# joaospinto/sip_optimal_control

Hardware: AMD Instinct MI355X
Metric: Riccati sweeps/sec (backward+forward) (higher is better)
Workload: dtype f64

## Files before the change

### __graft_entry__.py

```python
import os
import re
import subprocess
import sys

ROOT = os.path.dirname(os.path.abspath(__file__))
CSRC = os.path.join(ROOT, "sip_optimal_control_amd", "csrc")
LIBDIR = os.path.join(ROOT, "sip_optimal_control_amd", "lib")
HIPCC = os.environ.get("HIPCC", "/opt/rocm/bin/hipcc")


def _digest(paths, extra=()):
    import hashlib
    h = hashlib.sha256()
    for x in extra:
        h.update(("\0arg:" + x).encode())
    for path in sorted(set(paths), key=lambda q: os.path.relpath(q, ROOT)):
        h.update(("\0file:" + os.path.relpath(path, ROOT) + "\0").encode())
        with open(path, "rb") as f:
            h.update(f.read())
    return h.hexdigest()


def _stale(target, digest):
    side = target + ".srchash"
# ... 205 lines not shown
    return _host_build(out, [src, os.path.join(ROOT, "tests", "cpp", "test_dropin.cpp"), hdr,
                             os.path.join(ROOT, "include", "sip_lqr_amd.h")],
                       ["g++", "-std=c++17", "-O2", "-D__HIP_PLATFORM_AMD__", src,
                        "-I", os.path.join(ROOT, "include"), "-I", os.path.join(rocm, "include"),
                        "-L", LIBDIR, "-lsip_lqr_amd", "-L", os.path.join(rocm, "lib"), "-lamdhip64",
                        "-Wl,-rpath,$ORIGIN/../sip_optimal_control_amd/lib",
                        "-Wl,-rpath," + os.path.join(rocm, "lib"), "-o", out], force)


def build_callback_provider_test(force=False):
    src = os.path.join(ROOT, "tests", "cpp", "test_callback_provider.cpp")
    hdrs = [os.path.join(ROOT, "include", "sip_optimal_control_amd", h)
            for h in ("callback_provider_dropin.hpp", "lqr_dropin.hpp")]
    out = os.path.join(ROOT, "tests", "cpp", "test_callback_provider")
    rocm = os.environ.get("ROCM_PATH", "/opt/rocm")
    return _host_build(out, [src] + hdrs + [os.path.join(ROOT, "include", h) for h in ("sip_kkt_amd.h", "sip_lqr_amd.h")],
                       ["g++", "-std=c++17", "-O2", "-D__HIP_PLATFORM_AMD__", src,
                        "-I", os.path.join(ROOT, "include"), "-I", os.path.join(rocm, "include"),
                        "-L", LIBDIR, "-lsip_lqr_amd", "-L", os.path.join(rocm, "lib"), "-lamdhip64",
                        "-Wl,-rpath,$ORIGIN/../../sip_optimal_control_amd/lib",
                        "-Wl,-rpath," + os.path.join(rocm, "lib"), "-o", out], force)


def build_kkt_lds_test(force=False):
    src = os.path.join(ROOT, "tests", "cpp", "test_kkt_lds.cpp")
    hdrs = [os.path.join(CSRC, h) for h in ("kkt_kernels.hpp", "kkt_chain_kernels.hpp", "kkt_theta_kernels.hpp",
                                            "kkt_theta_chain_kernels.hpp", "kkt_chain_launch.hpp")]
    out = os.path.join(ROOT, "build", "test_kkt_lds")
    os.makedirs(os.path.dirname(out), exist_ok=True)
    return _host_build(out, [src] + hdrs,
                       [HIPCC, "-x", "hip", "--cuda-host-only", "-std=c++17", "-O1", src, "-o", out], force)


def build_kkt_plan_test(force=False):
    src = os.path.join(ROOT, "tests", "cpp", "test_kkt_plan.cpp")
    hdrs = [os.path.join(CSRC, h) for h in ("kkt_plan.hpp", "kkt_first_order_kernels.hpp", "kkt_kernels.hpp",
                                            "kkt_chain_kernels.hpp", "kkt_theta_kernels.hpp",
                                            "kkt_theta_chain_kernels.hpp", "kkt_chain_launch.hpp")]
    hdrs += [os.path.join(ROOT, "include", h) for h in ("sip_kkt_amd.h", "sip_lqr_amd.h")]
    out = os.path.join(ROOT, "build", "test_kkt_plan")
    os.makedirs(os.path.dirname(out), exist_ok=True)
    return _host_build(out, [src] + hdrs,
                       [HIPCC, "-x", "hip", "--offload-arch=gfx950", "-std=c++17", "-O1", src, "-o", out], force)


def build_tree_plan_test(force=False):
    src = os.path.join(ROOT, "tests", "cpp", "test_tree_plan.cpp")
    hdrs = [os.path.join(CSRC, h) for h in ("tree_plan.hpp", "generic_plan.hpp", "table_packer.hpp", "stream_fill.hpp",
                                            "tree_generic.hpp", "tree_lds.hpp", "tree_qw16_launch.hpp",
                                            "tree_schedule.hpp")]
    hdrs.append(os.path.join(ROOT, "include", "sip_lqr_amd.h"))
    out = os.path.join(ROOT, "build", "test_tree_plan")
    os.makedirs(os.path.dirname(out), exist_ok=True)
    return _host_build(out, [src] + hdrs,
                       [HIPCC, "-x", "hip", "--cuda-host-only", "-std=c++17", "-O1", src,
                        "-L", LIBDIR, "-lsip_lqr_amd", "-Wl,-rpath,$ORIGIN/../sip_optimal_control_amd/lib",
                        "-o", out], force)


def build_residual_cols_shape_test(force=False):
    src = os.path.join(ROOT, "tests", "cpp", "test_residual_cols_shape.cpp")
    out = os.path.join(ROOT, "build", "test_residual_cols_shape")
    os.makedirs(os.path.dirname(out), exist_ok=True)
    return _host_build(out, [src, os.path.join(CSRC, "residual_cols_shape.hpp")],
                       ["g++", "-std=c++17", "-O1", "-Wall", "-I", CSRC, src, "-o", out], force)


def build_tree_residual_cols_shape_test(force=False):
    src = os.path.join(ROOT, "tests", "cpp", "test_tree_residual_cols_shape.cpp")
    out = os.path.join(ROOT, "build", "test_tree_residual_cols_shape")
    os.makedirs(os.path.dirname(out), exist_ok=True)
    return _host_build(out, [src, os.path.join(CSRC, "tree_residual_cols_shape.hpp")],
                       ["g++", "-std=c++17", "-O1", "-Wall", "-I", CSRC, src, "-o", out], force)


def build_oracle():
    sys.path.insert(0, ROOT)
    from oracle import oracle
    return oracle.build()


def build():
    build_hip()
    build_rccl()
    build_group_test()
    build_dropin_test()
    build_dropin_split_test()
    build_callback_provider_test()
    build_kkt_lds_test()
    build_kkt_plan_test()
    build_tree_plan_test()
    build_residual_cols_shape_test()
    build_tree_residual_cols_shape_test()
    build_oracle()
    sys.path.insert(0, ROOT)
    import sip_optimal_control_amd
    from sip_optimal_control_amd._lib import load_library
    load_library()


def smoke():
    sys.path.insert(0, ROOT)
    import numpy as np
    import torch
    from sip_optimal_control_amd import BatchedChainLQR, ChainShape, synthetic
    from oracle import oracle
    assert torch.cuda.is_available(), "smoke() needs a GPU"
    from sip_optimal_control_amd._lib import load_library
    print("library:", load_library().sip_lqr_version().decode())
    shape = ChainShape(n=12, m=4, T=10)
    batch = 37
    mats, vecs = synthetic.make_chain_batch(shape, batch, seed=3, device="cuda:0", cross_term=0.01)
    solver = BatchedChainLQR(shape.n, shape.m, shape.T, batch, device="cuda:0")
    sol, gains, status = solver.factor_solve(mats, vecs)
    torch.cuda.synchronize()
    ref_sol, ref_gains, ref_status = oracle.chain_batch(shape.n, shape.m, shape.T,
                                                       mats.cpu().numpy(), vecs.cpu().numpy())
    assert (status.cpu().numpy() == ref_status).all(), "status mismatch"
    err = np.abs(sol.cpu().numpy() - ref_sol).max() / np.abs(ref_sol).max()
    gerr = np.abs(gains.cpu().numpy() - ref_gains).max() / np.abs(ref_gains).max()
    assert err < 1e-9 and gerr < 1e-9, (err, gerr)
    print(f"smoke ok: kernel={solver.kernel_name} rel err sol={err:.2e} gains={gerr:.2e}")
# ... 24 lines not shown
```

### sip_optimal_control_amd/csrc/chain_mt16.hip

```cpp
#include "chain_mt16.hpp"
#include "mt16_launch.hpp"

namespace sipamd {

static_assert(mt16::Layout<float, 8>::WSN == kMt16SpillPerNode && mt16::Layout<double, 4>::WSN == kMt16SpillPerNode,
              "the dispatch table sizes the workspace by kMt16SpillPerNode");

#define SIP_MT16_INSTANTIATE(S, M)                                                                           \
  template hipError_t launch_mt16<S, M>(long, int, const void *, const void *, void *, void *, int32_t *,    \
                                        void *, hipStream_t, int, void *);
SIP_MT16_INSTANTIATE(float, 8)
SIP_MT16_INSTANTIATE(float, 4)
SIP_MT16_INSTANTIATE(double, 8)
SIP_MT16_INSTANTIATE(double, 4)

}
```

### sip_optimal_control_amd/csrc/chain_mt16.hpp

```cpp
#pragma once
#include <hip/hip_runtime.h>

#include "mt16_launch.hpp"

#ifdef SIP_MT16_STAMPS
#define SIP_MT16_STAMP_ARG , unsigned long long *__restrict__ stamps
#define SIP_MT16_STAMP(k)                                                                                     \
  do {                                                                                                       \
    const unsigned long long now_ = __builtin_amdgcn_s_memtime();                                            \
    seg_[k] += now_ - last_;                                                                                 \
    last_ = now_;                                                                                            \
  } while (0)
#else
#define SIP_MT16_STAMP_ARG
#define SIP_MT16_STAMP(k)
#endif

namespace sipamd {
namespace mt16 {

constexpr int N = 32;

template <typename S> struct Tr;
template <> struct Tr<float> {
// ... 219 lines not shown
        ig = sel(L.mg[0], i0, sel(L.mg[1], i1, sel(L.mg[2], i2, i3)));
      } else {
        const S t1 = fma_(m10, L.eg[0], L.eg[1]);
        const S t2 = fma_(m20, L.eg[0], fma_(m21, L.eg[1], L.eg[2]));
        const S t3 = fma_(m30, L.eg[0], fma_(m31, L.eg[1], fma_(m32, L.eg[2], L.eg[3])));
        amix = fma_(L.ej[0], L.eg[0], fma_(L.ej[1], t1, fma_(L.ej[2], t2, L.ej[3] * t3)));
        ig = fma_(i0, L.eg[0], fma_(i1, L.eg[1], fma_(i2, L.eg[2], i3 * L.eg[3])));
      }
      const bool diag = L.j == TR::row(L.g, v);
      const S one_d = diag ? S(1) : S(0);
      S bop[TILES], aop[TILES];
#pragma unroll
      for (int Jt = 0; Jt < TILES; ++Jt) {
        const S src = T[I][Jt][v] - (Jt == I ? one_d : S(0));
        const v4 mixed = TR::mfma(amix, src, zero4<S>());
        aop[Jt] = -mixed[0];
        bop[Jt] = mixed[0] * ig;
      }
#pragma unroll
      for (int It = 0; It < TILES; ++It)
#pragma unroll
        for (int Jt = 0; Jt < TILES; ++Jt)
          T[It][Jt] = TR::mfma(aop[It], bop[Jt], T[It][Jt]);
      T[I][I][v] -= S(2) * one_d;
    }
  }
  return fail;
}

template <typename S, int M> struct Layout {
  static constexpr int NODE = N * N + N;
  static constexpr int EDGE = N * N + 2 * N * M + M * M;
  static constexpr int VNODE = 2 * N, VEDGE = M, GAIN = M * N + M;
  static constexpr int WTILES = 3, WSN = WTILES * 256 + N;
  static constexpr int VM = (M + 3) / 4;
  static constexpr bool VEC_LOADS = Tr<S>::ROWS_CONTIGUOUS && (EDGE % 4 == 0);
};

template <typename S, bool VEC>
__device__ __forceinline__ Mat32<S> load32(const rsrc_t r, const unsigned ocol, const unsigned so) {
  constexpr unsigned ES = sizeof(S);
  Mat32<S> m;
#pragma unroll
  for (int I = 0; I < 2; ++I)
#pragma unroll
    for (int J = 0; J < 2; ++J) {
      if constexpr (VEC) {
        m.t[I][J] = Mem<S>::ld4(r, (ocol + (unsigned)(16 * J * N + 16 * I)) * ES, so * ES);
      } else {
#pragma unroll
        for (int v = 0; v < 4; ++v)
          m.t[I][J][v] = Mem<S>::ld(r, (ocol + (unsigned)(16 * J * N + 16 * I + Tr<S>::RSTEP * v)) * ES, so * ES);
      }
    }
  return m;
}

#ifndef SIP_MT16_WAVES_F32
#define SIP_MT16_WAVES_F32 4
#endif
template <typename S, int M> struct Waves {
  static constexpr int value = sizeof(S) == 8 ? 2 : M > 8 ? 3 : SIP_MT16_WAVES_F32;
};

template <typename S, int M>
__global__ __launch_bounds__(64) __attribute__((amdgpu_waves_per_eu(Waves<S, M>::value, Waves<S, M>::value)))
void chain_factor_solve_mt16(
    const S *__restrict__ mats, const S *__restrict__ vecs, S *__restrict__ sol, S *__restrict__ gains,
    S *__restrict__ wsp, int *__restrict__ status, const long batch, const int T SIP_MT16_STAMP_ARG) {
  constexpr bool FACTOR = false;
// ... 45 lines not shown
```

### sip_optimal_control_amd/csrc/chain_mt16_solve.hip

```cpp
#include "chain_mt16_solve.hpp"
#include "mt16_launch.hpp"

namespace sipamd {

static_assert(mt16::Layout<float, 8>::WSN == kMt16SpillPerNode, "the spill the factor sweep left");
static_assert(mt16_col_workspace_scalars(3, 8, 5) == 4 * 5 * (mt16::N + 8), "cws[node][column][g | k]");

#define SIP_MT16_SOLVE_INSTANTIATE(S, M)                                                                     \
  template hipError_t launch_mt16_solve<S, M>(long, int, const void *, const void *, void *, void *, void *, \
                                              const void *, void *, const int32_t *, int, long, hipStream_t); \
  template hipError_t launch_mt16_factor<S, M>(long, int, const void *, void *, int32_t *, void *, void *, hipStream_t);
SIP_MT16_SOLVE_INSTANTIATE(float, 8)
SIP_MT16_SOLVE_INSTANTIATE(float, 4)
SIP_MT16_SOLVE_INSTANTIATE(double, 8)
SIP_MT16_SOLVE_INSTANTIATE(double, 4)

}
```

### sip_optimal_control_amd/csrc/chain_mt16_solve.hpp

```cpp
#pragma once
#include "chain_mt16.hpp"

namespace sipamd {
namespace mt16 {

template <typename S> __device__ __forceinline__ void mul_t_pair(const Mat32<S> &U, const Pair<S> &X, Pair<S> &acc) {
#pragma unroll
  for (int R = 0; R < 2; ++R)
#pragma unroll
    for (int v = 0; v < 4; ++v)
#pragma unroll
      for (int I = 0; I < 2; ++I)
        acc.t[I] = Tr<S>::mfma(U.t[R][I][v], X.t[R][v], acc.t[I]);
}

template <typename S, int M>
__global__ __launch_bounds__(64) __attribute__((amdgpu_waves_per_eu(2)))
void chain_solve_mt16(const S *__restrict__ mats, const S *__restrict__ vecs_cols, S *sol_cols, S *gains, S *wsp,
                      const S *__restrict__ gfac, S *cws, const int *__restrict__ status, const long batch,
                      const int T, const int ncols, const long col_stride) {
  static_assert(M >= 1 && M <= 16, "controls live in registers 0 .. VM - 1 of the four lane groups: 16 tile rows");
  using TR = Tr<S>;
  using v4 = typename TR::v4;
  using LY = Layout<S, M>;
  constexpr int STG = LY::NODE + LY::EDGE, VSTG = LY::VNODE + LY::VEDGE, VM = LY::VM;
  constexpr bool VEC = LY::VEC_LOADS;
  constexpr unsigned ES = sizeof(S);
  constexpr int GF = M * M + M;
  constexpr int CW = N + M;
  const long p = blockIdx.x;
  if (p >= batch || status[p] != 0)
    return;
  const int lane = threadIdx.x & 63, j = lane & 15, g = lane >> 4;
  const int acol = ctrl_of_col<S>(j);
  const bool colok = j < ncols;
  const long cj = colok ? j : 0;
  const long mats_len = (long)(T + 1) * LY::NODE + (long)T * LY::EDGE, vecs_len = (long)(T + 1) * LY::VNODE + (long)T * LY::VEDGE;
  const rsrc_t rM = make_rsrc(mats + p * mats_len, mats_len * ES);
  const rsrc_t rG = make_rsrc(gains + p * ((long)T * LY::GAIN), (long)T * LY::GAIN * ES);
  const rsrc_t rW = make_rsrc(wsp + p * ((long)(T + 1) * LY::WSN), (long)(T + 1) * LY::WSN * ES);
  const rsrc_t rF = make_rsrc(gfac + p * ((long)T * GF), (long)T * GF * ES);
  const S *pv = vecs_cols + cj * col_stride + p * vecs_len;
  S *ps = sol_cols + cj * col_stride + p * vecs_len;
  S *pg, *pk;
  long gstride, kstride;
  if (cws != nullptr) {
    pg = cws + (p * (long)(T + 1) * ncols + cj) * CW, gstride = (long)ncols * CW;
    pk = pg + N, kstride = gstride;
  } else {
    pg = wsp + p * ((long)(T + 1) * LY::WSN) + LY::WTILES * 256, gstride = LY::WSN;
    pk = gains + p * ((long)T * LY::GAIN) + M * N, kstride = LY::GAIN;
  }
  const unsigned acolc = (unsigned)(acol < M ? acol : 0);
  const unsigned uj = (unsigned)j, ug = (unsigned)g, r0 = (unsigned)TR::row(g, 0);
  const unsigned ocol = uj * N + r0;
  const unsigned obcol = acolc * N + r0;
  const unsigned orow = r0 * N + uj;
  const unsigned octl = ug * N + uj;
  auto ldM = [&](const unsigned vo, const unsigned so) { return Mem<S>::ld(rM, vo * ES, so * ES); };
  int arow[VM];
  bool aok[VM];
#pragma unroll
  for (int v = 0; v < VM; ++v) {
    const int a = ctrl_of(g, v);
    aok[v] = a < M, arow[v] = a < M ? a : M - 1;
  }

  auto ld_pair = [&](const S *base, const long off) {
    Pair<S> r;
#pragma unroll
    for (int I = 0; I < 2; ++I)
#pragma unroll
      for (int v = 0; v < 4; ++v) {
        const S x = base[off + 16 * I + TR::row(g, v)];
        r.t[I][v] = colok ? x : S(0);
      }
    return r;
  };
  auto st_pair = [&](S *base, const long off, const Pair<S> &x) {
    if (colok) {
#pragma unroll
      for (int I = 0; I < 2; ++I)
#pragma unroll
        for (int v = 0; v < 4; ++v)
          base[off + 16 * I + TR::row(g, v)] = x.t[I][v];
    }
  };
  auto ld_ctl = [&](const S *base, const long off) {
    v4 r = zero4<S>();
#pragma unroll
    for (int v = 0; v < VM; ++v) {
      const S x = base[off + arow[v]];
      r[v] = (colok && aok[v]) ? x : S(0);
    }
    return r;
  };
  auto st_ctl = [&](S *base, const long off, const v4 x) {
#pragma unroll
    for (int v = 0; v < VM; ++v)
      if (colok && aok[v])
        base[off + arow[v]] = x[v];
  };
  auto ld_delta = [&](const int i) {
    Pair<S> r;
#pragma unroll
    for (int I = 0; I < 2; ++I)
#pragma unroll
      for (int v = 0; v < 4; ++v)
        r.t[I][v] = ldM((unsigned)(N * N + 16 * I) + r0 + (unsigned)(TR::RSTEP * v), (unsigned)i * STG);
    return r;
  };
  auto fetch_W = [&](const int i) {
    Mat32<S> W;
    const unsigned sW = (unsigned)i * LY::WSN * ES, vl = (unsigned)lane * 4u * ES;
    W.t[0][0] = Mem<S>::ld4(rW, vl, sW), W.t[1][0] = Mem<S>::ld4(rW, vl + 256u * ES, sW);
    W.t[1][1] = Mem<S>::ld4(rW, vl + 512u * ES, sW);
    const unsigned gq = TR::ROWS_CONTIGUOUS ? (uj >> 2) : (uj & 3u), vq = TR::ROWS_CONTIGUOUS ? (uj & 3u) : (uj >> 2);
    const unsigned ot = (16u * gq + r0) * 4u + vq;
#pragma unroll
    for (int v = 0; v < 4; ++v)
      W.t[0][1][v] = Mem<S>::ld(rW, (ot + (unsigned)((64 + TR::RSTEP * v) * 4)) * ES, sW);
    return W;
  };
  auto t_of = [&](const Pair<S> &c, const Pair<S> &dl, const Pair<S> &v) {
    Pair<S> t;
#pragma unroll
    for (int I = 0; I < 2; ++I)
#pragma unroll
      for (int r = 0; r < 4; ++r)
        t.t[I][r] = fma_(-dl.t[I][r], v.t[I][r], c.t[I][r]);
    return t;
  };

  Mat32<S> W, A;
  Pair<S> B, K, q, c, dl;
  v4 Gm, rv;
  auto fetch_B = [&](const int i) {
    const unsigned sB = (unsigned)i * STG + LY::NODE + N * N;
#pragma unroll
    for (int I = 0; I < 2; ++I) {
      if constexpr (VEC) {
        B.t[I] = Mem<S>::ld4(rM, (obcol + (unsigned)(16 * I)) * ES, sB * ES);
      } else {
#pragma unroll
        for (int v = 0; v < 4; ++v)
          B.t[I][v] = ldM(obcol + (unsigned)(16 * I + TR::RSTEP * v), sB);
      }
      if (acol >= M)
        B.t[I] = zero4<S>();
    }
    rv = ld_ctl(pv, (long)i * VSTG + LY::VNODE);
  };
  auto fetch_G = [&](const int i) {
    Gm = zero4<S>();
#pragma unroll
    for (int v = 0; v < VM; ++v) {
// ... 169 lines not shown
```

### sip_optimal_control_amd/csrc/chain_mt16_sweep_body.hpp

```cpp
#ifndef SIP_MT16_SWEEP_BODY
#error "chain_mt16_sweep_body.hpp is the text of the two kernels of chain_mt16.hpp: include it only where they do"
#endif
  static_assert(M >= 1 && M <= 16, "controls live in registers 0 .. VM - 1 of the four lane groups: 16 tile rows");
#ifdef SIP_MT16_STAMPS
  unsigned long long seg_[16] = {0}, last_ = __builtin_amdgcn_s_memtime();
  const unsigned long long start_ = last_;
#endif
  using TR = Tr<S>;
  using v4 = typename TR::v4;
  using LY = Layout<S, M>;
  constexpr int STG = LY::NODE + LY::EDGE, VSTG = LY::VNODE + LY::VEDGE, VM = LY::VM;
  constexpr bool VEC = LY::VEC_LOADS;
  const long p = blockIdx.x;
  if (p >= batch)
    return;
  LaneT<S> L;
  L.lane = threadIdx.x & 63, L.j = L.lane & 15, L.g = L.lane >> 4;
#pragma unroll
  for (int k = 0; k < 4; ++k) {
    if constexpr (sizeof(S) == 4) {
      L.mg[k] = opaque_mask(L.g == k);
      L.mj[k] = opaque_mask(L.j == TR::row(k, 0));
    } else {
      L.eg[k] = L.g == k ? S(1) : S(0);
      L.ej[k] = L.j == TR::row(k, 0) ? S(1) : S(0);
    }
  }
  const int j = L.j, g = L.g;
  const int acol = ctrl_of_col<S>(j);
  constexpr unsigned ES = sizeof(S);
  const long mats_len = (long)(T + 1) * LY::NODE + (long)T * LY::EDGE, vecs_len = (long)(T + 1) * LY::VNODE + (long)T * LY::VEDGE;
  const rsrc_t rM = make_rsrc(mats + p * mats_len, mats_len * ES), rV = make_rsrc(vecs + p * vecs_len, vecs_len * ES);
  const rsrc_t rS = make_rsrc(sol + p * vecs_len, vecs_len * ES);
  const rsrc_t rG = make_rsrc(gains + p * ((long)T * LY::GAIN), (long)T * LY::GAIN * ES);
  const rsrc_t rW = make_rsrc(wsp + p * ((long)(T + 1) * LY::WSN), (long)(T + 1) * LY::WSN * ES);
  const unsigned acolc = (unsigned)(acol < M ? acol : 0);
  const unsigned uj = (unsigned)j, ug = (unsigned)g, r0 = (unsigned)TR::row(g, 0);
  const unsigned ocol = uj * N + r0;
  const unsigned obcol = acolc * N + r0;
  const unsigned orow = r0 * N + uj;
  const unsigned octl = ug * N + uj;
  constexpr unsigned RS = (unsigned)TR::RSTEP;
  auto ldM = [&](const unsigned vo, const unsigned so) { return Mem<S>::ld(rM, vo * ES, so * ES); };
  auto ldV = [&](const unsigned vo, const unsigned so) { return Mem<S>::ld(rV, vo * ES, so * ES); };

  constexpr int MH = M <= 8 ? 8 : 16;
  __shared__ S s_v[N], s_t[N], s_g[N], s_sd[N], s_sdi[N], s_x[N], s_z[N], s_gs[16], s_h[MH], s_u[MH];
  constexpr int LDM = TR::ROWS_CONTIGUOUS ? 36 : 33;
  __shared__ __attribute__((aligned(16))) S s_m[N * LDM];
  __shared__ __attribute__((aligned(16))) S s_p[16];


  if constexpr (!FACTOR) {
    if (L.lane < MH)
      s_h[L.lane] = S(0), s_u[L.lane] = S(0);
  }
  int stat = 0;
  Mat32<S> W, V;

  auto finish_node = [&](const int i, const S dl0, const S dl1, const S c0, const S c1) {
    if (stat == 0 && __any(!(dl0 > S(0)) || !(dl1 > S(0))))
      stat = 1;
    const S sd0 = TR::sqrt(dl0), sd1 = TR::sqrt(dl1);
    const S sdi0 = S(1) / sd0, sdi1 = S(1) / sd1;
    if (g == 0) {
      s_sd[j] = sd0, s_sd[16 + j] = sd1;
      s_sdi[j] = sdi0, s_sdi[16 + j] = sdi1;
      if constexpr (!FACTOR) {
        s_t[j] = c0 - dl0 * s_v[j];
        s_t[16 + j] = c1 - dl1 * s_v[16 + j];
      }
    }
    SIP_MT16_STAMP(7);
#pragma unroll
// ... 52 lines not shown
      for (int I = 0; I < 2; ++I)
#pragma unroll
        for (int J = 0; J < 2; ++J)
#pragma unroll
          for (int v = 0; v < 4; ++v)
            V.t[I][J][v] *= fr[I][v] * (J == 0 ? fs0 : fs1);
      const bool ffail_scaled = sweep<S, 2, 4>(V.t, L, s_p);
#pragma unroll
      for (int I = 0; I < 2; ++I)
#pragma unroll
        for (int J = 0; J < 2; ++J)
#pragma unroll
          for (int v = 0; v < 4; ++v)
            V.t[I][J][v] *= fr[I][v] * (J == 0 ? fs0 : fs1);
      if (stat == 0 && ffail_scaled)
        stat = 2;
    }
    const bool ffail = SCALE_F ? false : sweep<S, 2, 4>(V.t, L, s_p);
    SIP_MT16_STAMP(9);
    if (stat == 0 && ffail)
      stat = 2;
    {
      const v4 ir[2] = {by_row<S>(s_sdi, 0, g), by_row<S>(s_sdi, 1, g)};
#pragma unroll
      for (int I = 0; I < 2; ++I)
#pragma unroll
        for (int J = 0; J < 2; ++J)
#pragma unroll
          for (int v = 0; v < 4; ++v) {
            const bool dg = I == J && j == TR::row(g, v);
            W.t[I][J][v] = (V.t[I][J][v] + (dg ? S(1) : S(0))) * (ir[I][v] * (J == 0 ? sdi0 : sdi1));
          }
    }
    {
      const unsigned so = (unsigned)i * LY::WSN * ES, vo = (unsigned)L.lane * 4u * ES;
      Mem<S>::st4(W.t[0][0], rW, vo, so);
      Mem<S>::st4(W.t[1][0], rW, vo + 256u * ES, so);
      Mem<S>::st4(W.t[1][1], rW, vo + 512u * ES, so);
    }
    lds_order();
    SIP_MT16_STAMP(10);
  };

  {
    const unsigned sM = (unsigned)T * STG, sV = (unsigned)T * VSTG;
    V = load32<S, VEC>(rM, ocol, sM);
    if constexpr (!FACTOR) {
      const S qT0 = ldV(uj, sV), qT1 = ldV(uj + 16u, sV);
      if (g == 0)
        s_v[j] = qT0, s_v[16 + j] = qT1;
    }
    const S dl0 = ldM(uj + (unsigned)(N * N), sM), dl1 = ldM(uj + (unsigned)(N * N + 16), sM);
    S c0 = S(0), c1 = S(0);
    if constexpr (!FACTOR)
      c0 = ldV(uj + (unsigned)N, sV), c1 = ldV(uj + (unsigned)(N + 16), sV);
    lds_order();
    finish_node(T, dl0, dl1, c0, c1);
  }

  for (int i = T - 1; i >= 0; --i) {
    const unsigned sN = (unsigned)i * STG, sE = sN + LY::NODE, sB = sE + N * N, sMm = sB + N * M, sR = sMm + N * M;
    const unsigned sV = (unsigned)i * VSTG;
    const Mat32<S> A = load32<S, VEC>(rM, ocol, sE);
    const S dl0 = ldM(uj + (unsigned)(N * N), sN), dl1 = ldM(uj + (unsigned)(N * N + 16), sN);
    S c0 = S(0), c1 = S(0), q0 = S(0), q1 = S(0), rv = S(0);
    if constexpr (!FACTOR) {
      c0 = ldV(uj + (unsigned)N, sV), c1 = ldV(uj + (unsigned)(N + 16), sV);
      q0 = ldV(uj, sV), q1 = ldV(uj + 16u, sV), rv = ldV(acolc + (unsigned)LY::VNODE, sV);
    }
    Pair<S> B;
#pragma unroll
    for (int I = 0; I < 2; ++I) {
// ... 1 lines not shown
        B.t[I] = Mem<S>::ld4(rM, (obcol + (unsigned)(16 * I)) * ES, sB * ES);
      } else {
#pragma unroll
        for (int v = 0; v < 4; ++v)
          B.t[I][v] = ldM(obcol + (unsigned)(16 * I) + RS * v, sB);
      }
      if (acol >= M)
        B.t[I] = zero4<S>();
    }
    Pair<S> H;
    v4 G;
#pragma unroll
    for (int v = 0; v < 4; ++v) {
      const int a = ctrl_of(g, v);
      const bool ok = v < VM && a < M;
      if (v < VM) {
        const S h0 = ldM(octl + (unsigned)(4 * v * N), sMm), h1 = ldM(octl + (unsigned)(4 * v * N + 16), sMm);
        const S rr = ldM(acolc * M + ug + (unsigned)(4 * v), sR);
        H.t[0][v] = ok ? h0 : S(0);
        H.t[1][v] = ok ? h1 : S(0);
        G[v] = (ok && acol < M) ? rr : (j == TR::row(g, v) ? S(1) : S(0));
      } else {
        H.t[0][v] = S(0), H.t[1][v] = S(0);
        G[v] = j == TR::row(g, v) ? S(1) : S(0);
      }
    }
    if constexpr (!FACTOR) {
      const v4 tr[2] = {by_row<S>(s_t, 0, g), by_row<S>(s_t, 1, g)};
      S w0 = S(0), w1 = S(0);
      mat_t_vec<S>(W, tr, w0, w1);
      const S g0 = s_v[j] + sum_groups(w0), g1 = s_v[16 + j] + sum_groups(w1);
      if (g == 0) {
        s_g[j] = g0, s_g[16 + j] = g1;
        const unsigned so = ((unsigned)(i + 1) * LY::WSN + LY::WTILES * 256) * ES;
        Mem<S>::st(g0, rW, uj * ES, so);
        Mem<S>::st(g1, rW, (uj + 16u) * ES, so);
      }
    }
    SIP_MT16_STAMP(0);
    Mat32<S> F;
    Pair<S> Z;
#pragma unroll
    for (int I = 0; I < 2; ++I) {
      Z.t[I] = zero4<S>();
#pragma unroll
      for (int J = 0; J < 2; ++J)
        F.t[I][J] = zero4<S>();
    }
#pragma unroll
    for (int R = 0; R < 2; ++R)
#pragma unroll
      for (int v = 0; v < 4; ++v)
#pragma unroll
        for (int I = 0; I < 2; ++I) {
          Z.t[I] = TR::mfma(W.t[R][I][v], B.t[R][v], Z.t[I]);
#pragma unroll
          for (int J = 0; J < 2; ++J)
            F.t[I][J] = TR::mfma(W.t[R][I][v], A.t[R][J][v], F.t[I][J]);
        }
#pragma unroll
    for (int R = 0; R < 2; ++R)
#pragma unroll
      for (int v = 0; v < 4; ++v) {
        G = TR::mfma(B.t[R][v], Z.t[R][v], G);
        H.t[0] = TR::mfma(B.t[R][v], F.t[R][0][v], H.t[0]);
        H.t[1] = TR::mfma(B.t[R][v], F.t[R][1][v], H.t[1]);
      }
// ... 109 lines not shown
    lds_order();
    SIP_MT16_STAMP(5);
    finish_node(i, dl0, dl1, c0, c1);
  }
#ifdef SIP_MT16_STAMPS
  const unsigned long long back_end_ = __builtin_amdgcn_s_memtime();
#endif

  if constexpr (!FACTOR) {
    const v4 tr[2] = {by_row<S>(s_t, 0, g), by_row<S>(s_t, 1, g)};
    S w0 = S(0), w1 = S(0);
    mat_t_vec<S>(W, tr, w0, w1);
    const S g0 = s_v[j] + sum_groups(w0), g1 = s_v[16 + j] + sum_groups(w1);
    if (g == 0) {
      const S x0 = ldV(uj + (unsigned)N, 0u) - ldM(uj + (unsigned)(N * N), 0u) * g0;
      const S x1 = ldV(uj + (unsigned)(N + 16), 0u) - ldM(uj + (unsigned)(N * N + 16), 0u) * g1;
      Mem<S>::st(x0, rS, uj * ES, 0u), Mem<S>::st(x1, rS, (uj + 16u) * ES, 0u);
      Mem<S>::st(g0, rS, (uj + (unsigned)N) * ES, 0u), Mem<S>::st(g1, rS, (uj + (unsigned)(N + 16)) * ES, 0u);
      s_x[j] = x0, s_x[16 + j] = x1;
    }
  }
  if (L.lane == 0)
    status[p] = stat;
  lds_order();

  if constexpr (!FACTOR) {
  Pair<S> KT;
  Mat32<S> AT;
  Pair<S> BT;
  Mat32<S> Wc;
  S kb, gc0, gc1, cc0, cc1, dc0, dc1;
  auto fetch_K = [&](const int i) {
    const unsigned so = (unsigned)i * LY::GAIN * ES;
#pragma unroll
    for (int I = 0; I < 2; ++I)
#pragma unroll
      for (int v = 0; v < 4; ++v)
        KT.t[I][v] = Mem<S>::ld(rG, (r0 * M + acolc + (unsigned)((16 * I + TR::RSTEP * v) * M)) * ES, so);
    kb = Mem<S>::ld(rG, (acolc + (unsigned)(M * N)) * ES, so);
  };
  auto fetch_AB = [&](const int i) {
    const unsigned sE = (unsigned)i * STG + LY::NODE;
#pragma unroll
    for (int I = 0; I < 2; ++I)
#pragma unroll
      for (int v = 0; v < 4; ++v) {
        AT.t[I][0][v] = ldM(orow + (unsigned)((16 * I + TR::RSTEP * v) * N), sE);
        AT.t[I][1][v] = ldM(orow + (unsigned)((16 * I + TR::RSTEP * v) * N + 16), sE);
      }
#pragma unroll
    for (int v = 0; v < VM; ++v) {
      const int a = ctrl_of(g, v);
      const S b0 = ldM(octl + (unsigned)(N * N + 4 * v * N), sE), b1 = ldM(octl + (unsigned)(N * N + 4 * v * N + 16), sE);
      BT.t[0][v] = a < M ? b0 : S(0);
      BT.t[1][v] = a < M ? b1 : S(0);
    }
  };
  auto fetch_W = [&](const int i) {
    const unsigned sN1 = (unsigned)(i + 1) * STG, sV1 = (unsigned)(i + 1) * VSTG, sW = (unsigned)(i + 1) * LY::WSN;
    const unsigned vl = (unsigned)L.lane * 4u * ES;
    Wc.t[0][0] = Mem<S>::ld4(rW, vl, sW * ES), Wc.t[1][0] = Mem<S>::ld4(rW, vl + 256u * ES, sW * ES);
    Wc.t[1][1] = Mem<S>::ld4(rW, vl + 512u * ES, sW * ES);
    {
      const unsigned gq = TR::ROWS_CONTIGUOUS ? (uj >> 2) : (uj & 3u), vq = TR::ROWS_CONTIGUOUS ? (uj & 3u) : (uj >> 2);
      const unsigned ot = (16u * gq + r0) * 4u + vq;
#pragma unroll
      for (int v = 0; v < 4; ++v)
        Wc.t[0][1][v] = Mem<S>::ld(rW, (ot + (unsigned)((64 + TR::RSTEP * v) * 4)) * ES, sW * ES);
    }
    gc0 = Mem<S>::ld(rW, (uj + (unsigned)(LY::WTILES * 256)) * ES, sW * ES);
    gc1 = Mem<S>::ld(rW, (uj + (unsigned)(LY::WTILES * 256 + 16)) * ES, sW * ES);
    cc0 = ldV(uj + (unsigned)N, sV1), cc1 = ldV(uj + (unsigned)(N + 16), sV1);
    dc0 = ldM(uj + (unsigned)(N * N), sN1), dc1 = ldM(uj + (unsigned)(N * N + 16), sN1);
  };
  if (T > 0) {
    fetch_K(0);
    fetch_AB(0);
    fetch_W(0);
  }
  for (int i = 0; i < T; ++i) {
    const bool more = i + 1 < T;
    const v4 xr[2] = {by_row<S>(s_x, 0, g), by_row<S>(s_x, 1, g)};
    S pu = S(0);
#pragma unroll
    for (int I = 0; I < 2; ++I)
#pragma unroll
      for (int v = 0; v < 4; ++v)
        pu = fma_(KT.t[I][v], xr[I][v], pu);
    const S ub = kb + sum_groups(pu);
    if (more)
      fetch_K(i + 1);
    if (g == 0 && acol < M)
      s_u[acol] = ub;
    lds_order();
    S z0 = S(0), z1 = S(0);
    mat_t_vec<S>(AT, xr, z0, z1);
#pragma unroll
    for (int v = 0; v < VM; ++v) {
      const S ur = s_u[ctrl_of(g, v)];
      z0 = fma_(BT.t[0][v], ur, z0);
      z1 = fma_(BT.t[1][v], ur, z1);
    }
    if (more)
      fetch_AB(i + 1);
    z0 = sum_groups(z0), z1 = sum_groups(z1);
    if (g == 0)
// ... 29 lines not shown
```

### sip_optimal_control_amd/csrc/chain_mt16_wide.hip

```cpp
#include "chain_mt16.hpp"
#include "mt16_launch.hpp"

namespace sipamd {

static_assert(mt16::Layout<float, 16>::WSN == kMt16SpillPerNode && mt16::Layout<double, 12>::WSN == kMt16SpillPerNode,
              "the dispatch table sizes the workspace by kMt16SpillPerNode");
static_assert(mt16::Layout<double, 12>::VM == 3 && mt16::Layout<float, 16>::VM == 4, "control registers per lane");

#define SIP_MT16_WIDE_INSTANTIATE(S, M)                                                                      \
  template hipError_t launch_mt16<S, M>(long, int, const void *, const void *, void *, void *, int32_t *,    \
                                        void *, hipStream_t, int, void *);
SIP_MT16_WIDE_INSTANTIATE(float, 16)
SIP_MT16_WIDE_INSTANTIATE(float, 12)
SIP_MT16_WIDE_INSTANTIATE(double, 16)
SIP_MT16_WIDE_INSTANTIATE(double, 12)

}
```

### sip_optimal_control_amd/csrc/chain_mt16_wide_solve.hip

```cpp
#include "chain_mt16_solve.hpp"
#include "mt16_launch.hpp"

namespace sipamd {

static_assert(mt16::Layout<float, 16>::WSN == kMt16SpillPerNode, "the spill the factor sweep left");
static_assert(mt16_col_workspace_scalars(3, 16, 5) == 4 * 5 * (mt16::N + 16), "cws[node][column][g | k]");

#define SIP_MT16_WIDE_SOLVE_INSTANTIATE(S, M)                                                                \
  template hipError_t launch_mt16_solve<S, M>(long, int, const void *, const void *, void *, void *, void *, \
                                              const void *, void *, const int32_t *, int, long, hipStream_t); \
  template hipError_t launch_mt16_factor<S, M>(long, int, const void *, void *, int32_t *, void *, void *, hipStream_t);
SIP_MT16_WIDE_SOLVE_INSTANTIATE(float, 16)
SIP_MT16_WIDE_SOLVE_INSTANTIATE(float, 12)
SIP_MT16_WIDE_SOLVE_INSTANTIATE(double, 16)
SIP_MT16_WIDE_SOLVE_INSTANTIATE(double, 12)

}
```

### sip_optimal_control_amd/csrc/mt16_launch.hpp

```cpp
#pragma once
#include <hip/hip_runtime.h>

#include <cstdint>

namespace sipamd {

template <typename S, int M>
hipError_t launch_mt16(long batch, int T, const void *mats, const void *vecs, void *sol, void *gains,
                       int32_t *status, void *ws, hipStream_t stream, int mode, void *gfac);

constexpr int kMt16SpillPerNode = 3 * 256 + 32;

constexpr int kMt16SolveColumns = 16;
constexpr long mt16_col_workspace_scalars(int T, int m, int ncols) { return (long)(T + 1) * ncols * (32 + m); }
constexpr char kSeparateSuffix[] = " + chain_factor_mt16 + chain_solve_mt16";

template <typename S, int M>
hipError_t launch_mt16_factor(long batch, int T, const void *mats, void *gains, int32_t *status, void *ws, void *gfac,
                              hipStream_t stream);
template <typename S, int M>
hipError_t launch_mt16_solve(long batch, int T, const void *mats, const void *vecs_cols, void *sol_cols, void *gains,
                             void *ws, const void *gfac, void *cws, const int32_t *status, int ncols, long col_stride,
                             hipStream_t stream);

}

#define MT16_ENTRY(DT, S, TAG, M)                                                                            \
  sipamd::with_separate_sweeps({DT, 32, M, "chain_factor_solve_mt16<32," #M ",mfma16x16x4>/" TAG,            \
                                sipamd::kMt16SpillPerNode, &sipamd::launch_mt16<S, M>},                      \
                               {&sipamd::launch_mt16_factor<S, M>, &sipamd::launch_mt16_solve<S, M>,         \
                                sipamd::kSeparateSuffix, sipamd::kMt16SolveColumns, 32 + M})
```

Measured before the change: 13.24 million.

## Pack symmetric diagonal spill tiles for fp32 and hoist per-lane load offsets

Changes the per-node workspace spill of the symmetric W matrix. In fp32 the two diagonal 16x16 tiles are stored packed, keeping only one triangle (160 instead of 256 scalars each), and readers mirror the dropped entries from the transposed position. fp64 keeps the whole-tile layout. Load offsets in the forward sweep are pinned into registers with an empty asm barrier so the constant parts fold into immediates. The aim is less spill traffic and fewer address computations, at the cost of more complex indexing and an out-of-range store offset for dropped elements.

Result: slower. 12.99 million (-1.9%).

```diff
diff --git a/__graft_entry__.py b/__graft_entry__.py
--- a/__graft_entry__.py
+++ b/__graft_entry__.py
@@ -261,6 +261,15 @@
                        [HIPCC, "-x", "hip", "--cuda-host-only", "-std=c++17", "-O1", src, "-o", out], force)
 
 
+def build_mt16_spill_layout_test(force=False):
+    src = os.path.join(ROOT, "tests", "cpp", "test_mt16_spill_layout.cpp")
+    hdrs = [os.path.join(CSRC, h) for h in ("chain_mt16.hpp", "mt16_launch.hpp")]
+    out = os.path.join(ROOT, "build", "test_mt16_spill_layout")
+    os.makedirs(os.path.dirname(out), exist_ok=True)
+    return _host_build(out, [src] + hdrs,
+                       [HIPCC, "-x", "hip", "--cuda-host-only", "-std=c++17", "-O1", src, "-o", out], force)
+
+
 def build_kkt_plan_test(force=False):
     src = os.path.join(ROOT, "tests", "cpp", "test_kkt_plan.cpp")
     hdrs = [os.path.join(CSRC, h) for h in ("kkt_plan.hpp", "kkt_first_order_kernels.hpp", "kkt_kernels.hpp",
@@ -317,6 +326,7 @@
     build_dropin_split_test()
     build_callback_provider_test()
     build_kkt_lds_test()
+    build_mt16_spill_layout_test()
     build_kkt_plan_test()
     build_tree_plan_test()
     build_residual_cols_shape_test()
diff --git a/sip_optimal_control_amd/csrc/chain_mt16.hip b/sip_optimal_control_amd/csrc/chain_mt16.hip
--- a/sip_optimal_control_amd/csrc/chain_mt16.hip
+++ b/sip_optimal_control_amd/csrc/chain_mt16.hip
@@ -3,8 +3,10 @@
 
 namespace sipamd {
 
-static_assert(mt16::Layout<float, 8>::WSN == kMt16SpillPerNode && mt16::Layout<double, 4>::WSN == kMt16SpillPerNode,
-              "the dispatch table sizes the workspace by kMt16SpillPerNode");
+static_assert(mt16::Layout<float, 8>::WSN == mt16::spill_per_node<float>() && mt16::Layout<double, 4>::WSN == mt16::spill_per_node<double>(),
+              "the dispatch table sizes the workspace by mt16::spill_per_node");
+static_assert(mt16::Layout<float, 8>::WSN == 2 * 160 + 256 + 32 && mt16::Layout<double, 4>::WSN == 3 * 256 + 32,
+              "fp32: two packed diagonal tiles and tile (1, 0) | g; fp64: three whole tiles | g");
 
 #define SIP_MT16_INSTANTIATE(S, M)                                                                           \
   template hipError_t launch_mt16<S, M>(long, int, const void *, const void *, void *, void *, int32_t *,    \
diff --git a/sip_optimal_control_amd/csrc/chain_mt16.hpp b/sip_optimal_control_amd/csrc/chain_mt16.hpp
--- a/sip_optimal_control_amd/csrc/chain_mt16.hpp
+++ b/sip_optimal_control_amd/csrc/chain_mt16.hpp
@@ -275,10 +275,64 @@
   static constexpr int NODE = N * N + N;
   static constexpr int EDGE = N * N + 2 * N * M + M * M;
   static constexpr int VNODE = 2 * N, VEDGE = M, GAIN = M * N + M;
-  static constexpr int WTILES = 3, WSN = WTILES * 256 + N;
+  using SP = Spill<Tr<S>::ROWS_CONTIGUOUS>;
+  static constexpr bool PACKED = SP::PACKED;
+  static constexpr int WTILES = SP::WTILES, WSN = SP::WSN;
+  static constexpr int T00 = SP::T00, T10 = SP::T10, T11 = SP::T11, GOFF = SP::GOFF;
+  static __host__ __device__ constexpr bool kept(const int r, const int c) { return SP::kept(r, c); }
+  static __host__ __device__ constexpr int woff(const int r, const int c) { return SP::woff(r, c); }
+  static __host__ __device__ constexpr int roff(const int r, const int c) { return SP::roff(r, c); }
   static constexpr int VM = (M + 3) / 4;
   static constexpr bool VEC_LOADS = Tr<S>::ROWS_CONTIGUOUS && (EDGE % 4 == 0);
 };
+
+constexpr unsigned SPILL_DROPPED = 0x7ffff000u;
+template <typename S, int M> __device__ __forceinline__ unsigned spill_diag_offset(const int j, const int g) {
+  using LY = Layout<S, M>;
+  const int r = Tr<S>::row(g, 0);
+  return LY::kept(r, j) ? (unsigned)LY::woff(r, j) * (unsigned)sizeof(S) : SPILL_DROPPED;
+}
+template <typename S, int M>
+__device__ __forceinline__ void store_spill_W(const Mat32<S> &W, const rsrc_t rW, const unsigned so, const unsigned vdiag,
+                                              const int lane) {
+  using LY = Layout<S, M>;
+  constexpr unsigned ES = sizeof(S);
+  Mem<S>::st4(W.t[0][0], rW, vdiag + (unsigned)LY::T00 * ES, so);
+  Mem<S>::st4(W.t[1][0], rW, (unsigned)lane * 4u * ES + (unsigned)LY::T10 * ES, so);
+  Mem<S>::st4(W.t[1][1], rW, vdiag + (unsigned)LY::T11 * ES, so);
+}
+__device__ __forceinline__ unsigned in_place(unsigned x) {
+  asm volatile("" : "+v"(x));
+  return x;
+}
+template <typename S, int M>
+__device__ __forceinline__ Mat32<S> load_spill_W(const rsrc_t rW, const unsigned so, const int lane, const int j, const int g) {
+  using LY = Layout<S, M>;
+  using TR = Tr<S>;
+  constexpr unsigned ES = sizeof(S);
+  Mat32<S> W;
+  const unsigned vl = in_place((unsigned)lane * 4u * ES);
+  const unsigned vt = in_place((unsigned)LY::roff(TR::row(g, 0), 16 + j) * ES);
+  W.t[1][0] = Mem<S>::ld4(rW, vl + (unsigned)LY::T10 * ES, so);
+#pragma unroll
+  for (int v = 0; v < 4; ++v)
+    W.t[0][1][v] = Mem<S>::ld(rW, vt + (unsigned)(4 * TR::RSTEP * v) * ES, so);
+  if constexpr (LY::PACKED) {
+    const bool kp = LY::kept(TR::row(g, 0), j);
+    const unsigned vd = in_place((unsigned)(kp ? LY::woff(TR::row(g, 0), j) : LY::woff(j, TR::row(g, 0))) * ES);
+    const unsigned step = in_place(kp ? ES : 4u * ES);
+#pragma unroll
+    for (int v = 0; v < 4; ++v) {
+      const unsigned vo = vd + (unsigned)v * step;
+      W.t[0][0][v] = Mem<S>::ld(rW, vo + (unsigned)LY::T00 * ES, so);
+      W.t[1][1][v] = Mem<S>::ld(rW, vo + (unsigned)LY::T11 * ES, so);
+    }
+  } else {
+    W.t[0][0] = Mem<S>::ld4(rW, vl + (unsigned)LY::T00 * ES, so);
+    W.t[1][1] = Mem<S>::ld4(rW, vl + (unsigned)LY::T11 * ES, so);
+  }
+  return W;
+}
 
 template <typename S, bool VEC>
 __device__ __forceinline__ Mat32<S> load32(const rsrc_t r, const unsigned ocol, const unsigned so) {
diff --git a/sip_optimal_control_amd/csrc/chain_mt16_solve.hip b/sip_optimal_control_amd/csrc/chain_mt16_solve.hip
--- a/sip_optimal_control_amd/csrc/chain_mt16_solve.hip
+++ b/sip_optimal_control_amd/csrc/chain_mt16_solve.hip
@@ -3,7 +3,7 @@
 
 namespace sipamd {
 
-static_assert(mt16::Layout<float, 8>::WSN == kMt16SpillPerNode, "the spill the factor sweep left");
+static_assert(mt16::Layout<float, 8>::WSN == mt16::spill_per_node<float>(), "the spill the factor sweep left");
 static_assert(mt16_col_workspace_scalars(3, 8, 5) == 4 * 5 * (mt16::N + 8), "cws[node][column][g | k]");
 
 #define SIP_MT16_SOLVE_INSTANTIATE(S, M)                                                                     \
diff --git a/sip_optimal_control_amd/csrc/chain_mt16_solve.hpp b/sip_optimal_control_amd/csrc/chain_mt16_solve.hpp
--- a/sip_optimal_control_amd/csrc/chain_mt16_solve.hpp
+++ b/sip_optimal_control_amd/csrc/chain_mt16_solve.hpp
@@ -48,7 +48,7 @@
     pg = cws + (p * (long)(T + 1) * ncols + cj) * CW, gstride = (long)ncols * CW;
     pk = pg + N, kstride = gstride;
   } else {
-    pg = wsp + p * ((long)(T + 1) * LY::WSN) + LY::WTILES * 256, gstride = LY::WSN;
+    pg = wsp + p * ((long)(T + 1) * LY::WSN) + LY::GOFF, gstride = LY::WSN;
     pk = gains + p * ((long)T * LY::GAIN) + M * N, kstride = LY::GAIN;
   }
   const unsigned acolc = (unsigned)(acol < M ? acol : 0);
@@ -110,18 +110,7 @@
         r.t[I][v] = ldM((unsigned)(N * N + 16 * I) + r0 + (unsigned)(TR::RSTEP * v), (unsigned)i * STG);
     return r;
   };
-  auto fetch_W = [&](const int i) {
-    Mat32<S> W;
-    const unsigned sW = (unsigned)i * LY::WSN * ES, vl = (unsigned)lane * 4u * ES;
-    W.t[0][0] = Mem<S>::ld4(rW, vl, sW), W.t[1][0] = Mem<S>::ld4(rW, vl + 256u * ES, sW);
-    W.t[1][1] = Mem<S>::ld4(rW, vl + 512u * ES, sW);
-    const unsigned gq = TR::ROWS_CONTIGUOUS ? (uj >> 2) : (uj & 3u), vq = TR::ROWS_CONTIGUOUS ? (uj & 3u) : (uj >> 2);
-    const unsigned ot = (16u * gq + r0) * 4u + vq;
-#pragma unroll
-    for (int v = 0; v < 4; ++v)
-      W.t[0][1][v] = Mem<S>::ld(rW, (ot + (unsigned)((64 + TR::RSTEP * v) * 4)) * ES, sW);
-    return W;
-  };
+  auto fetch_W = [&](const int i) { return load_spill_W<S, M>(rW, (unsigned)i * LY::WSN * ES, lane, j, g); };
   auto t_of = [&](const Pair<S> &c, const Pair<S> &dl, const Pair<S> &v) {
     Pair<S> t;
 #pragma unroll
diff --git a/sip_optimal_control_amd/csrc/chain_mt16_sweep_body.hpp b/sip_optimal_control_amd/csrc/chain_mt16_sweep_body.hpp
--- a/sip_optimal_control_amd/csrc/chain_mt16_sweep_body.hpp
+++ b/sip_optimal_control_amd/csrc/chain_mt16_sweep_body.hpp
@@ -40,6 +40,7 @@
   const unsigned obcol = acolc * N + r0;
   const unsigned orow = r0 * N + uj;
   const unsigned octl = ug * N + uj;
+  const unsigned wdiag = spill_diag_offset<S, M>(j, g);
   constexpr unsigned RS = (unsigned)TR::RSTEP;
   auto ldM = [&](const unsigned vo, const unsigned so) { return Mem<S>::ld(rM, vo * ES, so * ES); };
   auto ldV = [&](const unsigned vo, const unsigned so) { return Mem<S>::ld(rV, vo * ES, so * ES); };
@@ -158,12 +159,7 @@
             W.t[I][J][v] = (V.t[I][J][v] + (dg ? S(1) : S(0))) * (ir[I][v] * (J == 0 ? sdi0 : sdi1));
           }
     }
-    {
-      const unsigned so = (unsigned)i * LY::WSN * ES, vo = (unsigned)L.lane * 4u * ES;
-      Mem<S>::st4(W.t[0][0], rW, vo, so);
-      Mem<S>::st4(W.t[1][0], rW, vo + 256u * ES, so);
-      Mem<S>::st4(W.t[1][1], rW, vo + 512u * ES, so);
-    }
+    store_spill_W<S, M>(W, rW, (unsigned)i * LY::WSN * ES, wdiag, L.lane);
     lds_order();
     SIP_MT16_STAMP(10);
   };
@@ -231,7 +227,7 @@
       const S g0 = s_v[j] + sum_groups(w0), g1 = s_v[16 + j] + sum_groups(w1);
       if (g == 0) {
         s_g[j] = g0, s_g[16 + j] = g1;
-        const unsigned so = ((unsigned)(i + 1) * LY::WSN + LY::WTILES * 256) * ES;
+        const unsigned so = ((unsigned)(i + 1) * LY::WSN + LY::GOFF) * ES;
         Mem<S>::st(g0, rW, uj * ES, so);
         Mem<S>::st(g1, rW, (uj + 16u) * ES, so);
       }
@@ -407,46 +403,41 @@
   S kb, gc0, gc1, cc0, cc1, dc0, dc1;
   auto fetch_K = [&](const int i) {
     const unsigned so = (unsigned)i * LY::GAIN * ES;
+    const unsigned vk = in_place((r0 * M + acolc) * ES), va = in_place(acolc * ES);
 #pragma unroll
     for (int I = 0; I < 2; ++I)
 #pragma unroll
       for (int v = 0; v < 4; ++v)
-        KT.t[I][v] = Mem<S>::ld(rG, (r0 * M + acolc + (unsigned)((16 * I + TR::RSTEP * v) * M)) * ES, so);
-    kb = Mem<S>::ld(rG, (acolc + (unsigned)(M * N)) * ES, so);
+        KT.t[I][v] = Mem<S>::ld(rG, vk + (unsigned)((16 * I + TR::RSTEP * v) * M) * ES, so);
+    kb = Mem<S>::ld(rG, va + (unsigned)(M * N) * ES, so);
   };
   auto fetch_AB = [&](const int i) {
     const unsigned sE = (unsigned)i * STG + LY::NODE;
+    const unsigned vr = in_place(orow * ES), vc = in_place(octl * ES);
 #pragma unroll
     for (int I = 0; I < 2; ++I)
 #pragma unroll
       for (int v = 0; v < 4; ++v) {
-        AT.t[I][0][v] = ldM(orow + (unsigned)((16 * I + TR::RSTEP * v) * N), sE);
-        AT.t[I][1][v] = ldM(orow + (unsigned)((16 * I + TR::RSTEP * v) * N + 16), sE);
+        AT.t[I][0][v] = Mem<S>::ld(rM, vr + (unsigned)((16 * I + TR::RSTEP * v) * N) * ES, sE * ES);
+        AT.t[I][1][v] = Mem<S>::ld(rM, vr + (unsigned)((16 * I + TR::RSTEP * v) * N + 16) * ES, sE * ES);
       }
 #pragma unroll
     for (int v = 0; v < VM; ++v) {
       const int a = ctrl_of(g, v);
-      const S b0 = ldM(octl + (unsigned)(N * N + 4 * v * N), sE), b1 = ldM(octl + (unsigned)(N * N + 4 * v * N + 16), sE);
+      const S b0 = Mem<S>::ld(rM, vc + (unsigned)(4 * v * N) * ES, (sE + (unsigned)(N * N)) * ES);
+      const S b1 = Mem<S>::ld(rM, vc + (unsigned)(4 * v * N + 16) * ES, (sE + (unsigned)(N * N)) * ES);
       BT.t[0][v] = a < M ? b0 : S(0);
       BT.t[1][v] = a < M ? b1 : S(0);
     }
   };
   auto fetch_W = [&](const int i) {
     const unsigned sN1 = (unsigned)(i + 1) * STG, sV1 = (unsigned)(i + 1) * VSTG, sW = (unsigned)(i + 1) * LY::WSN;
-    const unsigned vl = (unsigned)L.lane * 4u * ES;
-    Wc.t[0][0] = Mem<S>::ld4(rW, vl, sW * ES), Wc.t[1][0] = Mem<S>::ld4(rW, vl + 256u * ES, sW * ES);
-    Wc.t[1][1] = Mem<S>::ld4(rW, vl + 512u * ES, sW * ES);
-    {
-      const unsigned gq = TR::ROWS_CONTIGUOUS ? (uj >> 2) : (uj & 3u), vq = TR::ROWS_CONTIGUOUS ? (uj & 3u) : (uj >> 2);
-      const unsigned ot = (16u * gq + r0) * 4u + vq;
-#pragma unroll
-      for (int v = 0; v < 4; ++v)
-        Wc.t[0][1][v] = Mem<S>::ld(rW, (ot + (unsigned)((64 + TR::RSTEP * v) * 4)) * ES, sW * ES);
-    }
-    gc0 = Mem<S>::ld(rW, (uj + (unsigned)(LY::WTILES * 256)) * ES, sW * ES);
-    gc1 = Mem<S>::ld(rW, (uj + (unsigned)(LY::WTILES * 256 + 16)) * ES, sW * ES);
-    cc0 = ldV(uj + (unsigned)N, sV1), cc1 = ldV(uj + (unsigned)(N + 16), sV1);
-    dc0 = ldM(uj + (unsigned)(N * N), sN1), dc1 = ldM(uj + (unsigned)(N * N + 16), sN1);
+    Wc = load_spill_W<S, M>(rW, sW * ES, L.lane, j, g);
+    const unsigned vj = in_place(uj * ES);
+    gc0 = Mem<S>::ld(rW, vj + (unsigned)LY::GOFF * ES, sW * ES);
+    gc1 = Mem<S>::ld(rW, vj + (unsigned)(LY::GOFF + 16) * ES, sW * ES);
+    cc0 = Mem<S>::ld(rV, vj + (unsigned)N * ES, sV1 * ES), cc1 = Mem<S>::ld(rV, vj + (unsigned)(N + 16) * ES, sV1 * ES);
+    dc0 = Mem<S>::ld(rM, vj, (sN1 + (unsigned)(N * N)) * ES), dc1 = Mem<S>::ld(rM, vj + 16u * ES, (sN1 + (unsigned)(N * N)) * ES);
   };
   if (T > 0) {
     fetch_K(0);
diff --git a/sip_optimal_control_amd/csrc/chain_mt16_wide.hip b/sip_optimal_control_amd/csrc/chain_mt16_wide.hip
--- a/sip_optimal_control_amd/csrc/chain_mt16_wide.hip
+++ b/sip_optimal_control_amd/csrc/chain_mt16_wide.hip
@@ -3,8 +3,8 @@
 
 namespace sipamd {
 
-static_assert(mt16::Layout<float, 16>::WSN == kMt16SpillPerNode && mt16::Layout<double, 12>::WSN == kMt16SpillPerNode,
-              "the dispatch table sizes the workspace by kMt16SpillPerNode");
+static_assert(mt16::Layout<float, 16>::WSN == mt16::spill_per_node<float>() && mt16::Layout<double, 12>::WSN == mt16::spill_per_node<double>(),
+              "the dispatch table sizes the workspace by mt16::spill_per_node");
 static_assert(mt16::Layout<double, 12>::VM == 3 && mt16::Layout<float, 16>::VM == 4, "control registers per lane");
 
 #define SIP_MT16_WIDE_INSTANTIATE(S, M)                                                                      \
diff --git a/sip_optimal_control_amd/csrc/chain_mt16_wide_solve.hip b/sip_optimal_control_amd/csrc/chain_mt16_wide_solve.hip
--- a/sip_optimal_control_amd/csrc/chain_mt16_wide_solve.hip
+++ b/sip_optimal_control_amd/csrc/chain_mt16_wide_solve.hip
@@ -3,7 +3,7 @@
 
 namespace sipamd {
 
-static_assert(mt16::Layout<float, 16>::WSN == kMt16SpillPerNode, "the spill the factor sweep left");
+static_assert(mt16::Layout<float, 16>::WSN == mt16::spill_per_node<float>(), "the spill the factor sweep left");
 static_assert(mt16_col_workspace_scalars(3, 16, 5) == 4 * 5 * (mt16::N + 16), "cws[node][column][g | k]");
 
 #define SIP_MT16_WIDE_SOLVE_INSTANTIATE(S, M)                                                                \
diff --git a/sip_optimal_control_amd/csrc/mt16_launch.hpp b/sip_optimal_control_amd/csrc/mt16_launch.hpp
--- a/sip_optimal_control_amd/csrc/mt16_launch.hpp
+++ b/sip_optimal_control_amd/csrc/mt16_launch.hpp
@@ -9,7 +9,38 @@
 hipError_t launch_mt16(long batch, int T, const void *mats, const void *vecs, void *sol, void *gains,
                        int32_t *status, void *ws, hipStream_t stream, int mode, void *gfac);
 
-constexpr int kMt16SpillPerNode = 3 * 256 + 32;
+namespace mt16 {
+#if defined(__HIPCC__) || defined(__CUDACC__)
+#define SIP_MT16_HD __host__ __device__
+#else
+#define SIP_MT16_HD
+#endif
+template <bool ROWS_CONTIGUOUS> struct Spill {
+  static constexpr bool PACKED = ROWS_CONTIGUOUS;
+  static constexpr int WTILES = 3;
+  static constexpr int DIAG = PACKED ? 160 : 256;
+  static constexpr int T00 = 0, T10 = DIAG, T11 = DIAG + 256, GOFF = 2 * DIAG + 256;
+  static constexpr int WSN = GOFF + 32;
+  static SIP_MT16_HD constexpr int grp(const int rr) { return ROWS_CONTIGUOUS ? rr >> 2 : rr & 3; }
+  static SIP_MT16_HD constexpr int reg(const int rr) { return ROWS_CONTIGUOUS ? rr & 3 : rr >> 2; }
+  static SIP_MT16_HD constexpr int whole(const int rr, const int cc) { return (16 * grp(rr) + cc) * 4 + reg(rr); }
+  static SIP_MT16_HD constexpr int group(const int g, const int cc) {
+    const int b = cc >> 2;
+    return 4 * (4 * b - b * (b - 1) / 2) + 4 * (g - b) + (cc & 3);
+  }
+  static SIP_MT16_HD constexpr bool kept(const int r, const int c) {
+    const int I = r >> 4, J = c >> 4;
+    return I != J ? I > J : (!PACKED || 4 * grp(r & 15) + 3 >= (c & 15));
+  }
+  static SIP_MT16_HD constexpr int woff(const int r, const int c) {
+    const int I = r >> 4, rr = r & 15, cc = c & 15;
+    return I != (c >> 4) ? T10 + whole(rr, cc)
+                         : (I == 0 ? T00 : T11) + (PACKED ? group(grp(rr), cc) * 4 + reg(rr) : whole(rr, cc));
+  }
+  static SIP_MT16_HD constexpr int roff(const int r, const int c) { return kept(r, c) ? woff(r, c) : woff(c, r); }
+};
+template <typename S> constexpr int spill_per_node() { return Spill<sizeof(S) == 4>::WSN; }
+}
 
 constexpr int kMt16SolveColumns = 16;
 constexpr long mt16_col_workspace_scalars(int T, int m, int ncols) { return (long)(T + 1) * ncols * (32 + m); }
@@ -27,6 +58,6 @@
 
 #define MT16_ENTRY(DT, S, TAG, M)                                                                            \
   sipamd::with_separate_sweeps({DT, 32, M, "chain_factor_solve_mt16<32," #M ",mfma16x16x4>/" TAG,            \
-                                sipamd::kMt16SpillPerNode, &sipamd::launch_mt16<S, M>},                      \
+                                sipamd::mt16::spill_per_node<S>(), &sipamd::launch_mt16<S, M>},              \
                                {&sipamd::launch_mt16_factor<S, M>, &sipamd::launch_mt16_solve<S, M>,         \
                                 sipamd::kSeparateSuffix, sipamd::kMt16SolveColumns, 32 + M})
```
